# muyangyi/SimSeg

Hardware: AMD Instinct MI355X
Metric: image-text pairs/sec (train) + seg images/sec (eval), ViT-B (higher is better)
Workload: dtype fp16

## Files before the change

include/simseg_hip.h:

```cpp
#ifndef SIMSEG_HIP_H
#define SIMSEG_HIP_H
#include <stdint.h>
#ifdef __cplusplus
extern "C" {
#endif

int simseg_version(void);
int simseg_set_half_type(int t);
const char* simseg_last_error(void);

int simseg_gemm(const void* A, const void* B, void* C, int64_t M, int64_t N, int64_t K, int64_t lda, int64_t ldb,
                int64_t ldc, int in_dtype, int out_dtype, int transA, int transB, float alpha, const float* bias,
                const float* rowscale, const float* residual, int64_t ldr, int act, const void* aux, void* aux_out,
                int row_group, int res_mod, int accumulate, int splitk, uint64_t drop_seed, float drop_p, float* colsum,
                void* stream);
int simseg_gemm_aux_blocked_ok(int64_t M, int64_t N, int64_t K);

int simseg_patch_text_sim(const void* x, const void* text, float* out, int64_t M, int64_t C, int64_t K, int dtype, float eps,
                          int normalize, void* stream);

int simseg_set_gemm_variant(int v);
int simseg_gemm_last_variant(void);

int simseg_gemm_wgrad_group(const int64_t* problems, int n, int64_t rows, int slices, void* stream);
int simseg_wgrad_group_last(void);

int simseg_layernorm_fwd(const float* x, const float* gamma, const float* beta, void* y, int out_dtype, void* y_bf16,
                         float* mean, float* rstd, int64_t rows, int64_t D, float eps, void* stream);
int simseg_layernorm_bwd(const void* dy_bf16, const float* dy_f32, const float* dres, const void* dres_bf16, const float* x,
                         const void* y_bf16, const float* beta, const float* mean,
                         const float* rstd, const float* gamma, float* dx_f32, void* dx_bf16, float* dgamma,
                         float* dbeta, float* dxsum, float* partials, int64_t rows, int64_t D, uint64_t drop_seed, float drop_p,
                         void* stream);
int64_t simseg_layernorm_bwd_workspace_bytes(int64_t rows, int64_t D);

int simseg_colsum_accum(const void* in, int in_dtype, float* out, int64_t rows, int64_t N, int64_t ld, void* stream);

int simseg_vit_im2col(const float* image, void* cols, int out_dtype, int64_t B, int64_t H, int64_t W, void* stream);
int simseg_vit_cls_rows(const float* cls, const float* pos, float* x, int64_t B, int64_t T, int64_t D, void* stream);
int simseg_vit_cls_grad(const float* dx, float* dcls, int64_t B, int64_t T, int64_t D, void* stream);

int simseg_bert_embed_fwd(const int64_t* ids, const float* word, const float* pos, const float* type0, float* out,
                          int64_t B, int64_t L, int64_t D, int64_t vocab, void* stream);
int simseg_bert_embed_bwd(const int64_t* ids, const int64_t* mask, const float* dsum, float* dword, int64_t B, int64_t L,
                          int64_t D, int64_t vocab, void* stream);

int simseg_topk_pool_l2norm_fwd(const void* tok, int dtype, const int64_t* mask, float* emb, int32_t* idx, float* norm,
                                float* scratch, int64_t B, int64_t N, int64_t P, int k, float eps, int normalize, void* stream);
int64_t simseg_topk_pool_workspace_bytes(int64_t B, int64_t P, int k);
int simseg_topk_pool_l2norm_bwd(const float* demb, const float* emb, const float* norm, const int32_t* idx, void* dtok,
                                int dtype, int64_t B, int64_t N, int64_t P, int k, float eps, int normalize, void* stream);

int simseg_set_attention_variant(int v);
int simseg_debug_attn_trace(void* buf);
int simseg_debug_gemm_trace(void* buf);

// ... 153 lines not shown
```

simseg_amd/csrc/half_names.h:

```cpp
#pragma once
#ifdef SS_HALF
#define simseg_gemm_last_variant simseg_gemm_last_variant_h16
#define simseg_debug_gemm_trace simseg_debug_gemm_trace_h16
#define simseg_set_gemm_variant simseg_set_gemm_variant_h16
#define simseg_patch_text_sim simseg_patch_text_sim_h16
#define simseg_gemm_aux_blocked_ok simseg_gemm_aux_blocked_ok_h16
#define simseg_wgrad_group_last simseg_wgrad_group_last_h16
#define simseg_gemm_wgrad_group simseg_gemm_wgrad_group_h16
#define simseg_gemm simseg_gemm_h16
#define simseg_colsum_accum simseg_colsum_accum_h16
#define simseg_debug_attn_trace simseg_debug_attn_trace_h16
#define simseg_set_attention_variant simseg_set_attention_variant_h16
#define simseg_attention_fwd simseg_attention_fwd_h16
#define simseg_attention_fwd_qscaled simseg_attention_fwd_qscaled_h16
#define simseg_attention_fwd_x3 simseg_attention_fwd_x3_h16
#define simseg_debug_attention_timeline simseg_debug_attention_timeline_h16
#define simseg_attention_bwd_workspace_bytes simseg_attention_bwd_workspace_bytes_h16
#define simseg_attention_bwd simseg_attention_bwd_h16
#define simseg_attention_fwd_rows simseg_attention_fwd_rows_h16
#define simseg_attention_bwd_rows simseg_attention_bwd_rows_h16
#define simseg_attention_fwd_planes simseg_attention_fwd_planes_h16
#define simseg_attention_bwd_planes simseg_attention_bwd_planes_h16
#define simseg_layernorm_fwd simseg_layernorm_fwd_h16
#define simseg_layernorm_bwd simseg_layernorm_bwd_h16
#define simseg_layernorm_bwd_workspace_bytes simseg_layernorm_bwd_workspace_bytes_h16
#define simseg_vit_im2col simseg_vit_im2col_h16
#define simseg_topk_pool_workspace_bytes simseg_topk_pool_workspace_bytes_h16
#define simseg_topk_pool_l2norm_fwd simseg_topk_pool_l2norm_fwd_h16
#define simseg_topk_pool_l2norm_bwd simseg_topk_pool_l2norm_bwd_h16
#define simseg_row_rnorm simseg_row_rnorm_h16
#define simseg_cast simseg_cast_h16
#define simseg_dropout_apply simseg_dropout_apply_h16
#else
extern "C" {
int simseg_gemm_last_variant_h16(void);
int simseg_debug_gemm_trace_h16(void* buf);
int simseg_set_gemm_variant_h16(int v);
int simseg_patch_text_sim_h16(const void* x, const void* text, float* out, int64_t M, int64_t C, int64_t K, int dtype, float eps, int normalize, void* stream);
int simseg_gemm_aux_blocked_ok_h16(int64_t M, int64_t N, int64_t K);
int simseg_wgrad_group_last_h16(void);
int simseg_gemm_wgrad_group_h16(const int64_t* problems, int n, int64_t rows, int slices, void* stream);
int simseg_gemm_h16(const void* A, const void* B, void* C, int64_t M, int64_t N, int64_t K, int64_t lda, int64_t ldb, int64_t ldc, int in_dtype, int out_dtype, int transA, int transB, float alpha, const float* bias, const float* rowscale, const float* residual, int64_t ldr, int act, const void* aux, void* aux_out, int row_group, int res_mod, int accumulate, int splitk, uint64_t drop_seed, float drop_p, float* colsum, void* stream);
int simseg_colsum_accum_h16(const void* in, int in_dtype, float* out, int64_t rows, int64_t N, int64_t ld, void* stream);
int simseg_debug_attn_trace_h16(void* buf);
int simseg_set_attention_variant_h16(int v);
int simseg_attention_fwd_h16(const void* qkv, const int64_t* key_mask, void* out, float* lse, int dtype, int64_t B, int64_t T, int64_t H, float scale, uint64_t drop_seed, float drop_p, int skip_padded_rows, void* stream);
int simseg_attention_fwd_qscaled_h16(const void* qkv, void* out, float* lse, int64_t B, int64_t T, int64_t H, void* stream);
int simseg_attention_fwd_x3_h16(const void* qkv3, int64_t plane_elems, float* out, int64_t B, int64_t T, int64_t H, float scale, void* stream);
int simseg_debug_attention_timeline_h16(const void* qkv, void* out, float* lse, void* dbg, int64_t B, int64_t T, int64_t H, void* stream);
int64_t simseg_attention_bwd_workspace_bytes_h16(int64_t B, int64_t T, int64_t H);
int simseg_attention_bwd_h16(const void* qkv, const int64_t* key_mask, const void* out, const void* dout, const float* lse, float* workspace, void* dqkv, float* dqkv_colsum, int dtype, int64_t B, int64_t T, int64_t H, float scale, uint64_t drop_seed, float drop_p, int skip_padded_rows, void* stream);
int simseg_attention_fwd_rows_h16(const void* qkv, const int32_t* row_start, void* out, float* lse, int64_t B, int64_t T, int64_t H, float scale, uint64_t drop_seed, float drop_p, void* stream);
int simseg_attention_bwd_rows_h16(const void* qkv, const int32_t* row_start, const void* out, const void* dout, const float* lse, float* workspace, void* dqkv, float* dqkv_colsum, int64_t B, int64_t T, int64_t H, float scale, uint64_t drop_seed, float drop_p, void* stream);
int simseg_attention_fwd_planes_h16(const void* qkv, int64_t plane_rows, const int32_t* row_start, void* out, float* lse, int64_t B, int64_t T, int64_t H, float scale, uint64_t drop_seed, float drop_p, void* stream);
int simseg_attention_bwd_planes_h16(const void* qkv, int64_t plane_rows, const int32_t* row_start, const void* out, const void* dout, const float* lse, float* workspace, void* dqkv, float* dqkv_colsum, int64_t B, int64_t T, int64_t H, float scale, uint64_t drop_seed, float drop_p, void* stream);
int simseg_layernorm_fwd_h16(const float* x, const float* gamma, const float* beta, void* y, int out_dtype, void* y_bf16, float* mean, float* rstd, int64_t rows, int64_t D, float eps, void* stream);
int simseg_layernorm_bwd_h16(const void* dy_bf16, const float* dy_f32, const float* dres, const void* dres_bf16, const float* x, const void* y_bf16, const float* beta, const float* mean, const float* rstd, const float* gamma, float* dx_f32, void* dx_bf16, float* dgamma, float* dbeta, float* dxsum, float* partials, int64_t rows, int64_t D, uint64_t drop_seed, float drop_p, void* stream);
int64_t simseg_layernorm_bwd_workspace_bytes_h16(int64_t rows, int64_t D);
int simseg_vit_im2col_h16(const float* image, void* cols, int out_dtype, int64_t B, int64_t H, int64_t W, void* stream);
int64_t simseg_topk_pool_workspace_bytes_h16(int64_t B, int64_t P, int k);
int simseg_topk_pool_l2norm_fwd_h16(const void* tok, int dtype, const int64_t* mask, float* emb, int32_t* idx, float* norm, float* scratch, int64_t B, int64_t N, int64_t P, int k, float eps, int normalize, void* stream);
int simseg_topk_pool_l2norm_bwd_h16(const float* demb, const float* emb, const float* norm, const int32_t* idx, void* dtok, int dtype, int64_t B, int64_t N, int64_t P, int k, float eps, int normalize, void* stream);
int simseg_row_rnorm_h16(const void* x, int dtype, float* rnorm, int64_t rows, int64_t D, float eps, void* stream);
int simseg_cast_h16(const void* in, void* out, int64_t n, int to_bf16, void* stream);
int simseg_dropout_apply_h16(void* g, int dtype, int64_t n, uint64_t seed, float p, void* stream);
}
#endif
```

simseg_amd/csrc/rowops.hip:

```cpp
#include "common.h"
#include <atomic>
#include <stdlib.h>

namespace {

constexpr int LN_MAXC = 8;

typedef float f32x4_nt __attribute__((ext_vector_type(4)));
__device__ __forceinline__ void load4_nt(const float* p, float (&v)[4]) {
    const f32x4_nt t = __builtin_nontemporal_load(reinterpret_cast<const f32x4_nt*>(p));
    v[0] = t[0]; v[1] = t[1]; v[2] = t[2]; v[3] = t[3];
}
__device__ __forceinline__ void store4_nt(float* p, const float (&v)[4]) {
    const f32x4_nt t = {v[0], v[1], v[2], v[3]};
    __builtin_nontemporal_store(t, reinterpret_cast<f32x4_nt*>(p));
}

template <typename TO>
__global__ __launch_bounds__(256) void ln_fwd_kernel(const float* __restrict__ x, const float* __restrict__ gamma,
                                                     const float* __restrict__ beta, TO* __restrict__ y,
                                                     bf16_t* __restrict__ y2, float* __restrict__ mean_out,
                                                     float* __restrict__ rstd_out, int rows, int D, float eps) {
    const int lane = threadIdx.x & 63;
    const int row = __builtin_amdgcn_readfirstlane(blockIdx.x * 4 + (threadIdx.x >> 6));
// ... 369 lines not shown
                red[1][wave * 256 + lane * 4 + j] = ab[i][j];
                red[2][wave * 256 + lane * 4 + j] = as[i][j];
            }
        }
        __syncthreads();
        if (wave == 0 && (FULL || c < nch)) {
#pragma unroll
            for (int j = 0; j < 4; ++j) {
                float sg = 0.f, sb = 0.f, ss = 0.f;
                for (int w = 0; w < 4; ++w) { sg += red[0][w * 256 + lane * 4 + j]; sb += red[1][w * 256 + lane * 4 + j]; ss += red[2][w * 256 + lane * 4 + j]; }
                if (partials) {
                    float* pb = partials + (long)blockIdx.x * 3 * D + c * 4 + j;
                    pb[0] = sg; pb[D] = sb; pb[2 * D] = ss;
                } else {
                    atomicAdd(dgamma + c * 4 + j, sg);
                    atomicAdd(dbeta + c * 4 + j, sb);
                    if (dxsum) atomicAdd(dxsum + c * 4 + j, ss);
                }
            }
        }
    }
}

__global__ __launch_bounds__(256) void ln_bwd_reduce_kernel(const float* __restrict__ partials, int nblocks, int D, float* __restrict__ dgamma,
                                                            float* __restrict__ dbeta, float* __restrict__ dxsum) {
    const int col = blockIdx.x * 256 + threadIdx.x;
    if (col >= 3 * D) return;
    float* dst = col < D ? dgamma + col : (col < 2 * D ? dbeta + (col - D) : (dxsum ? dxsum + (col - 2 * D) : nullptr));
    if (!dst) return;
    const int per = (nblocks + gridDim.y - 1) / gridDim.y;
    const int b0 = blockIdx.y * per, b1 = min(nblocks, b0 + per);
    float s0 = 0.f, s1 = 0.f, s2 = 0.f, s3 = 0.f;
    int b = b0;
    for (; b + 4 <= b1; b += 4) {
        s0 += partials[(long)b * 3 * D + col];
        s1 += partials[(long)(b + 1) * 3 * D + col];
        s2 += partials[(long)(b + 2) * 3 * D + col];
        s3 += partials[(long)(b + 3) * 3 * D + col];
    }
    for (; b < b1; ++b) s0 += partials[(long)b * 3 * D + col];
    if (b1 > b0) atomicAdd(dst, (s0 + s1) + (s2 + s3));
}

template <typename TI>
__global__ __launch_bounds__(256) void colsum_kernel(const TI* __restrict__ in, float* __restrict__ out, long rows, int N,
                                                     long ld, int rows_per_block) {
// ... 216 lines not shown

__global__ void cast_f32_bf16_kernel(const float* __restrict__ in, bf16_t* __restrict__ out, long n4) {
    for (long i = (long)blockIdx.x * blockDim.x + threadIdx.x; i < n4; i += (long)gridDim.x * blockDim.x) {
        float v[4];
        load4<float>(in + i * 4, v);
        store4<bf16_t>(out + i * 4, v);
    }
}
__global__ void cast_bf16_f32_kernel(const bf16_t* __restrict__ in, float* __restrict__ out, long n4) {
    for (long i = (long)blockIdx.x * blockDim.x + threadIdx.x; i < n4; i += (long)gridDim.x * blockDim.x) {
        float v[4];
        load4<bf16_t>(in + i * 4, v);
        store4<float>(out + i * 4, v);
    }
}

template <typename T>
__global__ void dropout_apply_kernel(T* __restrict__ g, long n, unsigned long long seed, unsigned int thresh, float scale) {
    for (long i = (long)blockIdx.x * blockDim.x + threadIdx.x; i < n; i += (long)gridDim.x * blockDim.x)
        g[i] = (T)(dropout_keep(seed, (unsigned long long)i, thresh) ? (float)g[i] * scale : 0.f);
}

constexpr int LN_BWD_MAX_GRID = 2048;
inline int ln_bwd_grid(const void* fn, int slot, size_t lds, long rows) {
    constexpr int MAXDEV = 16;
    static std::atomic<int> ncu[MAXDEV];
    static std::atomic<unsigned long long> cached[MAXDEV][32];
    static std::atomic<int> forced{-1};
    int dev = 0;
    if (hipGetDevice(&dev) != hipSuccess || dev < 0 || dev >= MAXDEV) dev = 0;
    int n_cu = ncu[dev].load(std::memory_order_relaxed);
    if (n_cu <= 0) {
        n_cu = 256;
        hipDeviceProp_t prop;
        if (hipGetDeviceProperties(&prop, dev) == hipSuccess && prop.multiProcessorCount > 0) n_cu = prop.multiProcessorCount;
        ncu[dev].store(n_cu, std::memory_order_relaxed);
    }
    int f = forced.load(std::memory_order_relaxed);
    if (f < 0) {
        const char* e = getenv("SIMSEG_LN_BWD_BLOCKS_PER_CU");
        const int v = e ? atoi(e) : 0;
        f = v > 0 ? v : 0;
        forced.store(f, std::memory_order_relaxed);
    }
    const bool ok = slot >= 0 && slot < 32;
    const unsigned long long ent = ok ? cached[dev][slot].load(std::memory_order_relaxed) : 0ull;
    int per_cu = (ent != 0 && (ent >> 8) == (unsigned long long)lds) ? (int)(ent & 0xff) : 0;
    if (per_cu <= 0) {
        if (hipOccupancyMaxActiveBlocksPerMultiprocessor(&per_cu, fn, 256, lds) != hipSuccess || per_cu <= 0) { (void)hipGetLastError(); per_cu = 4; }
        if (per_cu > 255) per_cu = 255;
        if (ok) cached[dev][slot].store(((unsigned long long)lds << 8) | (unsigned long long)per_cu, std::memory_order_relaxed);
    }
    if (f > 0) per_cu = f;
    const long per_dev = (long)per_cu * n_cu;
    const int want = grid_for(rows, 4, LN_BWD_MAX_GRID);
    return want < per_dev ? want : (int)per_dev;
}

}

#define STREAM ((hipStream_t)stream)

extern "C" int simseg_layernorm_fwd(const float* x, const float* gamma, const float* beta, void* y, int out_dtype,
                                    void* y_bf16, float* mean, float* rstd, int64_t rows, int64_t D, float eps, void* stream) {
    SS_HALF_FWD(simseg_layernorm_fwd, x, gamma, beta, y, out_dtype, y_bf16, mean, rstd, rows, D, eps, stream);
    SS_CHECK(x && gamma && beta && y, "layernorm_fwd: null pointer");
    SS_CHECK(D % 4 == 0 && D <= LN_MAXC * 256 && D > 0, "layernorm_fwd: D=%lld must be a multiple of 4 and <= %d", (long long)D, LN_MAXC * 256);
    if (rows <= 0) return 0;
// ... 39 lines not shown
    } while (0)
#define LN_BWD16_LAUNCH(C, F)                                                                                                         \
    do {                                                                                                                              \
        grid = ln_bwd_grid((const void*)ln_bwd16_kernel<C, F>, C * 3 + (F ? 1 : 2), lds, rows);                                       \
        hipLaunchKernelGGL((ln_bwd16_kernel<C, F>), dim3(grid), dim3(256), lds, STREAM, (const bf16_t*)dy_bf16, (const bf16_t*)dres_bf16, x, (const bf16_t*)y_bf16, beta, mean, rstd, gamma, \
                           (bf16_t*)dx_bf16, dgamma, dbeta, dxsum, partials, (int)rows, (int)D, (unsigned long long)drop_seed, thresh, scale); \
    } while (0)
#define LN_BWD_PICK(C) do { if (!fast) LN_BWD_LAUNCH(C); else if (D == (C) * 256) LN_BWD16_LAUNCH(C, true); else LN_BWD16_LAUNCH(C, false); } while (0)
    if (nc <= 1) LN_BWD_PICK(1);
    else if (nc == 2) LN_BWD_PICK(2);
    else if (nc == 3) LN_BWD_PICK(3);
    else if (nc == 4) LN_BWD_PICK(4);
    else LN_BWD_PICK(8);
#undef LN_BWD_PICK
#undef LN_BWD16_LAUNCH
#undef LN_BWD_LAUNCH
    if (partials)
        hipLaunchKernelGGL(ln_bwd_reduce_kernel, dim3((unsigned)((3 * D + 255) / 256), 32), dim3(256), 0, STREAM, partials, grid, (int)D,
                           dgamma, dbeta, dxsum);
    SS_LAUNCH_CHECK("layernorm_bwd");
    return 0;
}

extern "C" int64_t simseg_layernorm_bwd_workspace_bytes(int64_t rows, int64_t D) { return (int64_t)grid_for(rows, 4, LN_BWD_MAX_GRID) * 3 * D * (int64_t)sizeof(float); }

extern "C" int simseg_colsum_accum(const void* in, int in_dtype, float* out, int64_t rows, int64_t N, int64_t ld, void* stream) {
    SS_HALF_FWD(simseg_colsum_accum, in, in_dtype, out, rows, N, ld, stream);
    SS_CHECK(in && out, "colsum: null pointer");
    SS_CHECK(N % 8 == 0 && ld % 8 == 0, "colsum: N and ld must be multiples of 8");
    if (rows <= 0) return 0;
    int chunks = (int)((rows + 255) / 256);
    if (chunks > 512) chunks = 512;
    const int nbx = (int)((N + 255) / 256);
    if ((long)chunks * nbx < 512) {
        const long by_rows = (rows + 7) / 8, by_grid = (512 + nbx - 1) / nbx;
        chunks = (int)(by_rows < by_grid ? by_rows : by_grid);
    }
    const int rpb = (int)((rows + chunks - 1) / chunks);
    dim3 grid((unsigned)nbx, (unsigned)((rows + rpb - 1) / rpb));
    if (in_dtype == 0)
        hipLaunchKernelGGL(colsum_kernel<float>, grid, dim3(256), 0, STREAM, (const float*)in, out, (long)rows, (int)N, (long)ld, rpb);
    else
        hipLaunchKernelGGL(colsum_kernel<bf16_t>, grid, dim3(256), 0, STREAM, (const bf16_t*)in, out, (long)rows, (int)N, (long)ld, rpb);
    SS_LAUNCH_CHECK("colsum");
    return 0;
}
// ... 109 lines not shown
```

simseg_amd/ops.py:

```python
import ctypes
import os
import threading

import torch

from .lib import call, ptr, require_gpu, stream, raw

F32, BF16 = 0, 1
_DT = {torch.float32: F32, torch.bfloat16: BF16, torch.float16: BF16}
HALF_TYPES = (torch.bfloat16, torch.float16)


def dt(t):
    try:
        return _DT[t.dtype]
    except KeyError:
        raise TypeError(f"simseg_amd supports fp32, bf16 and fp16 tensors, got {t.dtype}")


def _c(t):
    if t is not None and not t.is_contiguous():
        raise ValueError("simseg_amd ops need contiguous tensors")
    return t

# ... 155 lines not shown
    y16 = torch.empty(x.shape, device=x.device, dtype=want_bf16_copy if isinstance(want_bf16_copy, torch.dtype) else torch.bfloat16) if want_bf16_copy else None
    mean = torch.empty(rows, device=x.device, dtype=torch.float32) if save_stats else None
    rstd = torch.empty(rows, device=x.device, dtype=torch.float32) if save_stats else None
    call("simseg_layernorm_fwd", ptr(_c(x)), ptr(gamma), ptr(beta), ptr(y), dt(y), ptr(y16), ptr(mean), ptr(rstd), rows, D,
         float(eps), stream())
    return y, y16, mean, rstd


def layernorm_bwd(x, mean, rstd, gamma, dgamma, dbeta, dy16=None, dy32=None, dres=None, want_f32=True, want_bf16=True,
                  dxsum=None, drop_seed=0, drop_p=0.0, dres16=None, y16=None, beta=None):
    require_gpu(x)
    D = x.shape[-1]
    rows = x.numel() // D
    dx32 = torch.empty(x.shape, device=x.device, dtype=torch.float32) if want_f32 else None
    h16 = dy16.dtype if dy16 is not None else (want_bf16 if isinstance(want_bf16, torch.dtype) else torch.bfloat16)
    dx16 = torch.empty(x.shape, device=x.device, dtype=h16) if want_bf16 else None
    partials = torch.empty(raw("simseg_layernorm_bwd_workspace_bytes", rows, D) // 4, device=x.device, dtype=torch.float32)
    call("simseg_layernorm_bwd", ptr(_c(dy16)), ptr(_c(dy32)), ptr(_c(dres)), ptr(_c(dres16)), ptr(_c(x)), ptr(_c(y16)), ptr(_c(beta)) if y16 is not None else None,
         ptr(mean), ptr(rstd), ptr(gamma),
         ptr(dx32), ptr(dx16), ptr(dgamma), ptr(dbeta), ptr(dxsum), ptr(partials), rows, D, int(drop_seed), float(drop_p), stream())
    return dx32, dx16


def colsum_accum(x2d, out):
    require_gpu(x2d)
    call("simseg_colsum_accum", ptr(_c(x2d)), dt(x2d), ptr(out), x2d.shape[0], x2d.shape[1], x2d.shape[1], stream())
    return out


def vit_im2col(image, out_dtype):
    require_gpu(image)
    B, C, H, W = image.shape
    if C != 3 or image.dtype != torch.float32:
        raise ValueError("vit_im2col expects fp32 [B,3,H,W]")
    cols = torch.empty(B * (H // 16) * (W // 16), 768, device=image.device, dtype=out_dtype)
    call("simseg_vit_im2col", ptr(_c(image)), ptr(cols), dt(cols), B, H, W, stream())
    return cols


def vit_cls_rows(cls, pos, x):
    B, T, D = x.shape
    call("simseg_vit_cls_rows", ptr(cls), ptr(pos), ptr(x), B, T, D, stream())


def vit_cls_grad(dx, dcls):
    B, T, D = dx.shape
# ... 755 lines not shown
```

simseg_amd/towers.py:

```python
import contextlib
import os
import weakref

import torch
from torch.autograd import Function

from . import ops

BF16, F32 = torch.bfloat16, torch.float32


_W16 = {}


def weights_rewritten(param, w16):
    _W16[id(param)] = (weakref.ref(param), param._version, param.data_ptr(), w16)
    _W3.pop(id(param), None)
    for key in _WQS_OF.pop(id(param), ()):
        _WQS.pop(key, None)


def invalidate_weight_cache():
    _W16.clear()
    _CAT.clear()
# ... 127 lines not shown
        return cat
    return torch.cat(parts)


def _splitk(m, n, k_rows):
    tiles = ((m + 127) // 128) * ((n + 127) // 128)
    nk = (k_rows + 63) // 64
    return max(1, min(nk, (1024 + tiles - 1) // tiles, 64))


def _zeros(device, *shapes):
    sizes = [int(torch.Size(sh).numel()) if not isinstance(sh, int) else sh for sh in shapes]
    offs, o = [], 0
    for n in sizes:
        offs.append(o)
        o += (n + 63) // 64 * 64
    buf = torch.zeros(o, device=device, dtype=F32)
    return [buf[a:a + n].view(sh) for a, n, sh in zip(offs, sizes, shapes)]


_GELU8 = os.environ.get("SIMSEG_AMD_GELU_GRAD_BITS", "8") != "16"
_RES16 = os.environ.get("SIMSEG_AMD_RESGRAD_BITS", "16") != "32"
_XHAT_Y = os.environ.get("SIMSEG_AMD_LN_BWD_FROM_OUTPUT", "1") != "0"


def _lazy32(shape, device, dx16, dsum):
    dx = torch.empty(shape, device=device, dtype=F32)
    dx._simseg_lazy32 = True
    _put_shadow(dx, dx16.view(shape), dsum)
    return dx


def _need_shadow(t32, sh):
    if sh is None and getattr(t32, "_simseg_lazy32", False):
        raise RuntimeError("a residual-stream gradient that exists only as its 16-bit shadow (SIMSEG_AMD_RESGRAD_BITS=16) reached a consumer without a "
                           "valid shadow - was it modified in place, or consumed twice?  Set SIMSEG_AMD_RESGRAD_BITS=32")


def _grad_target(p):
    f = getattr(p, "_simseg_grad_target", None)
    return f() if f is not None else None


def _zeros_or(device, targets, *shapes):
    use = [t is not None and tuple(t.shape) == tuple(torch.Size(sh if not isinstance(sh, int) else (sh,))) for t, sh in zip(targets, shapes)]
    rest = iter(_zeros(device, *[sh for sh, u in zip(shapes, use) if not u]))
# ... 464 lines not shown
    try:
        mask._simseg_ragged = (mask._version, multiple, plan)
    except Exception:
        pass
    return plan


def ragged_maps(mask, multiple=256):
    p = ragged_plan(mask, multiple)
    return p.idx, p.inv, p.nv


def ragged_rows(mask):
    return ragged_plan(mask).cu


_PACKED_ATTN = os.environ.get("SIMSEG_AMD_PACKED_ATTN", "1") != "0"


class BertLayerFn(_GradAwareFn):

    @staticmethod
    def forward(ctx, x, mask, heads, adt, drop_p, seed, qw, qb, kw, kb, vw, vb, ow, ob, law, lab, iw, ib, o2w, o2b, low, lob, idx=None, inv=None,
                cu=None, nv=0):
        packed = idx is not None
        B, L = mask.shape
        D = x.shape[-1]
        x = x.contiguous()
        save = _saving(ctx)
        sh16 = getattr(x, "_simseg_fwd16", None) if adt != F32 else None
        if sh16 is not None and sh16[1] == x._version and sh16[0].numel() == x.numel():
            xa = sh16[0].view(-1, D)
        else:
            xa = x.view(-1, D) if adt == F32 else ops.cast(x.view(-1, D), adt)
        wqkv = _wt_stacked((qw, kw, vw), adt)
        bqkv = _as_one(qb.detach(), kb.detach(), vb.detach())
        if bqkv is None:
            bqkv = torch.cat([qb.detach(), kb.detach(), vb.detach()])
        ow_, iw_, o2w_ = _wt(ow, adt), _wt(iw, adt), _wt(o2w, adt)
        qkv = ops.gemm(xa, wqkv, bias=bqkv)
        rows = packed and cu is not None and adt != F32
        if rows:
            att, lse = ops.attention_fwd_rows(qkv, heads, cu, L, scale=64 ** -0.5, save_lse=save, drop_seed=seed, drop_p=drop_p, n_real=nv)
            attd = None
        else:
            if packed:
                qkv = ops.gather_rows(qkv, inv)
            att, lse = ops.attention_fwd(qkv.view(B, L, 3 * D), heads, mask, scale=64 ** -0.5, save_lse=save, drop_seed=seed, drop_p=drop_p,
                                          skip_padded_rows=packed and _SKIP_PAD, zero_skipped=False)
            attd = att
            if packed:
                att = ops.gather_rows(att.view(-1, D), idx)
        s1 = _fwd_gemm(att.view(-1, D), ow, adt, save, bias=ob.detach(), residual=x.view(-1, D), out_dtype=F32, drop_seed=seed + 1, drop_p=drop_p)
        a32, a16, mean_a, rstd_a = ops.layernorm_fwd(s1, law.detach(), lab.detach(), 1e-12, want_bf16_copy=(adt if adt != F32 else False), save_stats=save)
        aa = a32 if adt == F32 else a16
        blk = save and adt != F32 and ops.gemm_aux_blocked_ok(aa.shape[0], iw.shape[0], D)
        g8 = blk and _GELU8
        pre = torch.empty(x.shape[0] if packed else B * L, iw.shape[0], device=x.device, dtype=torch.uint8 if g8 else adt) if save else None
        act = _fwd_gemm(aa, iw, adt, save, bias=ib.detach(), act=((7 if g8 else 5) if blk else 3) if save else 1, aux_out=pre)
        s2 = _fwd_gemm(act, o2w, adt, save, bias=o2b.detach(), residual=a32, out_dtype=F32, drop_seed=seed + 2, drop_p=drop_p)
        y, y16, mean_o, rstd_o = ops.layernorm_fwd(s2, low.detach(), lob.detach(), 1e-12, want_bf16_copy=(adt if (adt != F32 and packed) else False), save_stats=save)
        if y16 is not None:
            y._simseg_fwd16 = (y16, y._version)
        ctx.adt, ctx.heads, ctx.dims, ctx.drop, ctx.packed, ctx.rows, ctx.nv, ctx.blk = adt, heads, (B, L, D), (drop_p, seed), packed, rows, nv, (2 if g8 else 1) if blk else 0
        ctx.wparams = (o2w, iw, ow)
        if save:
            ctx.save_for_backward(xa, mask, qkv, att, lse, s1, mean_a, rstd_a, aa, pre, act, s2, mean_o, rstd_o, wqkv, ow_, iw_, o2w_,
                                  law.detach(), low.detach(), attd if (packed and not rows) else None, idx, inv, cu if rows else None)
        return y if packed else y.view(B, L, D)

    @staticmethod
    @_joins_wgrad
    def backward(ctx, dy):
        (xa, mask, qkv, att, lse, s1, mean_a, rstd_a, aa, pre, act, s2, mean_o, rstd_o, wqkv, ow_, iw_, o2w_, law, low, attd, idx, inv, cu) = ctx.saved_tensors
        B, L, D = ctx.dims
        packed = ctx.packed
        adt = ctx.adt
        p, seed = ctx.drop
        need = ctx.needs_input_grad
        dy = dy.contiguous().view(-1, D)
        I = pre.shape[1]
        tg = [_grad_target(w) if nd else None for w, nd in zip(ctx.wparams, (need[18], need[16], need[12]))]
        (dlow, dlob, do2b, dib, do2w_z, diw_z, dlaw, dlab, dob, dow_z, dwqkv_z, dbqkv_z) = _zeros_or(
            dy.device, (None, None, None, None, tg[0], tg[1], None, None, None, tg[2], None, None),
            (D,), (D,), (D,), (I,), (D, I), (I, D), (D,), (D,), (D,), (D, D), (3 * D, D), (3 * D,))
        ds2_32, d2 = _ln_bwd(adt, s2, mean_o, rstd_o, low, dlow, dlob, None if adt != F32 else dy, dy32=dy if adt != F32 else None,
                             dxsum=do2b, drop=(p, seed + 2))
        group = [] if _wgrad_grouped(adt, (need[18], need[16], need[12], need[6] or need[8] or need[10])) else None
        wg = _wgrad if group is None else (lambda d, x_, z: group.append((d, x_, z)) or z)
        dpre = _dgrad(d2, o2w_, act=(4, 6, 8)[ctx.blk], aux=pre, colsum=dib)
        do2w = wg(d2, act, do2w_z) if need[18] else None
        da = _dgrad(dpre, iw_) if adt != F32 else _dgrad(dpre, iw_, residual=ds2_32)
        diw = wg(dpre, aa, diw_z) if need[16] else None
        ds1_32, d1 = _ln_bwd(adt, s1, mean_a, rstd_a, law, dlaw, dlab, da, dy32=ds2_32 if adt != F32 else None, dxsum=dob,
                             drop=(p, seed + 1))
        datt = _dgrad(d1, ow_)
        dow = wg(d1, att.view(-1, D), dow_z) if need[12] else None
        dbqkv = _zeros_like_bias(dbqkv_z, 3 * D, qkv.device) if (need[7] or need[9] or need[11]) else None
        if ctx.rows:
            dqkv = ops.attention_bwd_rows(qkv, att, datt.contiguous(), lse, ctx.heads, cu, L, scale=64 ** -0.5, drop_seed=seed, drop_p=p,
                                          colsum=dbqkv if _FUSED_QKV_BIAS else None, n_real=ctx.nv)
        else:
            if packed:
                datt = ops.gather_rows(datt, inv)
            dqkv = ops.attention_bwd(qkv.view(B, L, 3 * D), (attd if packed else att).view(B, L, D), datt.view(B, L, D), lse, ctx.heads, mask,
                                     scale=64 ** -0.5, drop_seed=seed, drop_p=p, skip_padded_rows=packed and _SKIP_PAD,
                                     colsum=dbqkv if _FUSED_QKV_BIAS else None, zero_skipped=False).view(-1, 3 * D)
            if packed:
                dqkv = ops.gather_rows(dqkv, idx)
        if dbqkv is not None and not _FUSED_QKV_BIAS:
            ops.colsum_accum(dqkv, dbqkv)
        dx = _dgrad(dqkv, wqkv, residual=ds1_32, out_dtype=F32)
        dwqkv = wg(dqkv, xa, dwqkv_z) if (need[6] or need[8] or need[10]) else None
        if group:
            _wgrad_flush(group)
        dws = [dwqkv[i * D:(i + 1) * D] if dwqkv is not None else None for i in range(3)]
        dbs = [dbqkv[i * D:(i + 1) * D] if dbqkv is not None else None for i in range(3)]
        return (dx if packed else dx.view(B, L, D), None, None, None, None, None, dws[0], dbs[0], dws[1], dbs[1], dws[2], dbs[2], dow, dob,
                dlaw, dlab, diw, dib, do2w, do2b, dlow, dlob, None, None, None, None)


_PACK_TEXT = [False, None]
_SKIP_PAD = os.environ.get("SIMSEG_AMD_SKIP_PAD_ROWS", "1") != "0"


@contextlib.contextmanager
def packed_text(lengths=None):
    prev = list(_PACK_TEXT)
    _PACK_TEXT[0] = os.environ.get("SIMSEG_AMD_PACKED_TEXT", "1") != "0"
    _PACK_TEXT[1] = lengths
    try:
        yield
    finally:
        _PACK_TEXT[:] = prev


def bert_forward(m, input_ids, attention_mask, adt, training=False, seed=0):
    p_h = m.hidden_dropout_prob if training else 0.0
    p_a = m.attention_probs_dropout_prob if training else 0.0
    if p_h != p_a:
        raise NotImplementedError("hidden and attention dropout probabilities are expected to be equal (HF default 0.1)")
    e = m.embeddings
    mask = attention_mask.contiguous().long()
    x = BertEmbedFn.apply(input_ids, mask, e.word_embeddings.weight, e.position_embeddings.weight, e.token_type_embeddings.weight,
                          e.LayerNorm.weight, e.LayerNorm.bias, p_h, seed)
    B, L, D = x.shape
    idx = inv = cu = None
    nv = 0
    if _PACK_TEXT[0] and x.is_cuda:
        lengths = _PACK_TEXT[1]
        plan = ragged_plan(mask, lengths=lengths if (lengths is not None and len(lengths) == B) else None)
        idx, inv, nv = plan.idx, plan.inv, plan.nv
        if nv == 0 or idx.numel() >= B * L:
            idx = inv = None
        else:
            x = RowMapFn.apply(x.view(-1, D), idx, inv)
            if _PACKED_ATTN and adt != F32 and L <= 256:
                cu = plan.cu
    for i, lyr in enumerate(m.encoder.layer):
        a, s = lyr.attention, lyr.attention.self
        x = BertLayerFn.apply(x, mask, m.num_heads, adt, p_h, seed + 16 * (i + 1),
                              s.query.weight, s.query.bias, s.key.weight, s.key.bias, s.value.weight, s.value.bias,
                              a.output.dense.weight, a.output.dense.bias, a.output.LayerNorm.weight, a.output.LayerNorm.bias,
                              lyr.intermediate.dense.weight, lyr.intermediate.dense.bias,
                              lyr.output.dense.weight, lyr.output.dense.bias, lyr.output.LayerNorm.weight, lyr.output.LayerNorm.bias,
                              idx, inv, cu, nv)
    if idx is not None:
        x = RowMapFn.apply(x, inv, idx).view(B, L, D)
    return x


_SKIP_MASKS = {}


def _skip_mask(B, N, skip, device):
    key = (B, N, skip, str(device))
    m = _SKIP_MASKS.get(key)
    if m is None:
        if len(_SKIP_MASKS) > 16:
            _SKIP_MASKS.clear()
        m = torch.ones(B, N, device=device, dtype=torch.int64)
        m[:, :skip] = 0
        _SKIP_MASKS[key] = m
    return m


class ProjectPoolFn(_GradAwareFn):

    @staticmethod
# ... 32 lines not shown
```

Before: 6150.

## Carry BERT residual gradients in 16-bit through a fused post-LN backward kernel

Adds a LayerNorm-backward kernel that takes one or two 16-bit gradient addends (or one fp32 addend), rebuilds xhat from the saved 16-bit LN output, and writes 16-bit dx plus an optional dropout-masked copy. The packed BERT text tower uses it so residual gradients stay in 16-bit between the two LayerNorms and across layers, and the fp32 dx of layers after the first is materialized lazily. The goal is less fp32 memory traffic in text-tower backward. The cost is lower precision in residual-gradient accumulation and more code paths, including shadow-gradient plumbing between layers.

```diff
diff --git a/include/simseg_hip.h b/include/simseg_hip.h
--- a/include/simseg_hip.h
+++ b/include/simseg_hip.h
@@ -32,6 +32,10 @@
                          const float* rstd, const float* gamma, float* dx_f32, void* dx_bf16, float* dgamma,
                          float* dbeta, float* dxsum, float* partials, int64_t rows, int64_t D, uint64_t drop_seed, float drop_p,
                          void* stream);
+int simseg_layernorm_bwd_post16(const void* dy_a, const void* dy_b, const float* dy_a_f32, const float* x, const void* y_bf16, const float* beta,
+                                const float* mean, const float* rstd, const float* gamma, void* dx_bf16, void* dxm_bf16,
+                                float* dx_f32, float* dgamma, float* dbeta, float* dxsum, float* partials, int64_t rows, int64_t D,
+                                uint64_t drop_seed, float drop_p, void* stream);
 int64_t simseg_layernorm_bwd_workspace_bytes(int64_t rows, int64_t D);
 
 int simseg_colsum_accum(const void* in, int in_dtype, float* out, int64_t rows, int64_t N, int64_t ld, void* stream);
diff --git a/simseg_amd/csrc/half_names.h b/simseg_amd/csrc/half_names.h
--- a/simseg_amd/csrc/half_names.h
+++ b/simseg_amd/csrc/half_names.h
@@ -23,6 +23,7 @@
 #define simseg_attention_bwd_planes simseg_attention_bwd_planes_h16
 #define simseg_layernorm_fwd simseg_layernorm_fwd_h16
 #define simseg_layernorm_bwd simseg_layernorm_bwd_h16
+#define simseg_layernorm_bwd_post16 simseg_layernorm_bwd_post16_h16
 #define simseg_layernorm_bwd_workspace_bytes simseg_layernorm_bwd_workspace_bytes_h16
 #define simseg_vit_im2col simseg_vit_im2col_h16
 #define simseg_topk_pool_workspace_bytes simseg_topk_pool_workspace_bytes_h16
@@ -56,6 +57,7 @@
 int simseg_attention_bwd_planes_h16(const void* qkv, int64_t plane_rows, const int32_t* row_start, const void* out, const void* dout, const float* lse, float* workspace, void* dqkv, float* dqkv_colsum, int64_t B, int64_t T, int64_t H, float scale, uint64_t drop_seed, float drop_p, void* stream);
 int simseg_layernorm_fwd_h16(const float* x, const float* gamma, const float* beta, void* y, int out_dtype, void* y_bf16, float* mean, float* rstd, int64_t rows, int64_t D, float eps, void* stream);
 int simseg_layernorm_bwd_h16(const void* dy_bf16, const float* dy_f32, const float* dres, const void* dres_bf16, const float* x, const void* y_bf16, const float* beta, const float* mean, const float* rstd, const float* gamma, float* dx_f32, void* dx_bf16, float* dgamma, float* dbeta, float* dxsum, float* partials, int64_t rows, int64_t D, uint64_t drop_seed, float drop_p, void* stream);
+int simseg_layernorm_bwd_post16_h16(const void* dy_a, const void* dy_b, const float* dy_a_f32, const float* x, const void* y_bf16, const float* beta, const float* mean, const float* rstd, const float* gamma, void* dx_bf16, void* dxm_bf16, float* dx_f32, float* dgamma, float* dbeta, float* dxsum, float* partials, int64_t rows, int64_t D, uint64_t drop_seed, float drop_p, void* stream);
 int64_t simseg_layernorm_bwd_workspace_bytes_h16(int64_t rows, int64_t D);
 int simseg_vit_im2col_h16(const float* image, void* cols, int out_dtype, int64_t B, int64_t H, int64_t W, void* stream);
 int64_t simseg_topk_pool_workspace_bytes_h16(int64_t B, int64_t P, int k);
diff --git a/simseg_amd/csrc/rowops.hip b/simseg_amd/csrc/rowops.hip
--- a/simseg_amd/csrc/rowops.hip
+++ b/simseg_amd/csrc/rowops.hip
@@ -415,6 +415,158 @@
     }
 }
 
+template <int MAXC, bool FULL, int ADD>
+__global__ __launch_bounds__(256) void ln_post16_kernel(const bf16_t* __restrict__ dya, const bf16_t* __restrict__ dyb, const float* __restrict__ dya32,
+                                                        const float* __restrict__ x, const bf16_t* __restrict__ y16, const float* __restrict__ beta,
+                                                        const float* __restrict__ mean, const float* __restrict__ rstd,
+                                                        const float* __restrict__ gamma, bf16_t* __restrict__ dx16, bf16_t* __restrict__ dxm16,
+                                                        float* __restrict__ dx32, float* __restrict__ dgamma,
+                                                        float* __restrict__ dbeta, float* __restrict__ dxsum, float* __restrict__ partials,
+                                                        int rows, int D,
+                                                        unsigned long long drop_seed, unsigned int drop_thresh, float drop_scale) {
+    constexpr bool TWO = ADD == 1, A32 = ADD == 2;
+    __shared__ float red[3][1024];
+    extern __shared__ float par[];
+    const int lane = threadIdx.x & 63, wave = threadIdx.x >> 6;
+    const int nch = D >> 2;
+    float ag[MAXC][4], ab[MAXC][4], as[MAXC][4];
+    unsigned okmask = 0;
+    int off[MAXC];
+#pragma unroll
+    for (int i = 0; i < MAXC; ++i) {
+#pragma unroll
+        for (int j = 0; j < 4; ++j) { ag[i][j] = 0.f; ab[i][j] = 0.f; as[i][j] = 0.f; }
+        const int c = lane + 64 * i;
+        off[i] = (FULL || c < nch) ? c * 4 : 0;
+        if (FULL || c < nch) {
+            float gm[4], bt[4], ig[4];
+            load4<float>(gamma + c * 4, gm);
+            load4<float>(beta + c * 4, bt);
+            bool ok = true;
+#pragma unroll
+            for (int j = 0; j < 4; ++j) { ok = ok && fabsf(gm[j]) >= 0.05f && fabsf(bt[j]) <= 4.f * fabsf(gm[j]); ig[j] = 1.0f / gm[j]; }
+            if (ok) okmask |= 1u << i;
+            if (wave == 0) { store4<float>(par + c * 4, gm); store4<float>(par + D + c * 4, ig); store4<float>(par + 2 * D + c * 4, bt); }
+        } else {
+            okmask |= 1u << i;
+        }
+    }
+    const bool needx = !__all(okmask == (1u << MAXC) - 1u);
+    __syncthreads();
+    const int stride = gridDim.x * 4;
+    int row = __builtin_amdgcn_readfirstlane(blockIdx.x * 4 + wave);
+    bf16x4 rda[A32 ? 1 : MAXC], rdb[TWO ? MAXC : 1], ry[MAXC];
+    f32x4_nt rdf[A32 ? MAXC : 1];
+#define LNP16_ISSUE(R)                                                                                            \
+    do {                                                                                                          \
+        const long ro_ = (long)(R) * D;                                                                           \
+        _Pragma("unroll") for (int i = 0; i < MAXC; ++i) {                                                        \
+            if (A32) rdf[A32 ? i : 0] = __builtin_nontemporal_load(reinterpret_cast<const f32x4_nt*>(dya32 + ro_ + off[i])); \
+            else rda[A32 ? 0 : i] = __builtin_nontemporal_load(reinterpret_cast<const bf16x4*>(dya + ro_ + off[i])); \
+            if (TWO) rdb[TWO ? i : 0] = __builtin_nontemporal_load(reinterpret_cast<const bf16x4*>(dyb + ro_ + off[i])); \
+            ry[i] = __builtin_nontemporal_load(reinterpret_cast<const bf16x4*>(y16 + ro_ + off[i]));              \
+        }                                                                                                         \
+    } while (0)
+    if (row < rows) LNP16_ISSUE(row);
+    for (; row < rows; row += stride) {
+        const float rs = rstd[row];
+        const long ro = (long)row * D;
+        float g[MAXC][4], xh[MAXC][4];
+        float s1 = 0.f, s2 = 0.f;
+        asm volatile("" ::: "memory");
+        if (needx) {
+            const float mu = mean[row];
+#pragma unroll
+            for (int i = 0; i < MAXC; ++i)
+                if (!((okmask >> i) & 1u)) {
+                    load4_nt(x + ro + off[i], xh[i]);
+#pragma unroll
+                    for (int j = 0; j < 4; ++j) xh[i][j] = (xh[i][j] - mu) * rs;
+                }
+        }
+        __builtin_amdgcn_sched_barrier(0);
+#pragma unroll
+        for (int i = 0; i < MAXC; ++i) {
+            const int c = lane + 64 * i;
+            const bool valid = FULL || c < nch;
+            const bool fromy = !needx || ((okmask >> i) & 1u);
+            float gm[4], ig[4], bt[4];
+            if (i) __builtin_amdgcn_sched_barrier(0);
+            load4<float>(par + off[i], gm);
+            load4<float>(par + D + off[i], ig);
+            load4<float>(par + 2 * D + off[i], bt);
+#pragma unroll
+            for (int j = 0; j < 4; ++j) {
+                const float sum = A32 ? rdf[A32 ? i : 0][j] : (TWO ? (float)rda[A32 ? 0 : i][j] + (float)rdb[TWO ? i : 0][j] : (float)rda[A32 ? 0 : i][j]);
+                const float a = valid ? sum : 0.f;
+                const float fy = ((float)ry[i][j] - bt[j]) * ig[j];
+                xh[i][j] = valid ? (fromy ? fy : xh[i][j]) : 0.f;
+                ag[i][j] += a * xh[i][j];
+                ab[i][j] += a;
+                g[i][j] = a * gm[j];
+                s1 += g[i][j];
+                s2 += g[i][j] * xh[i][j];
+            }
+        }
+        __builtin_amdgcn_sched_barrier(0);
+        { const int nr = row + stride < rows ? row + stride : row; LNP16_ISSUE(nr); }
+        __builtin_amdgcn_sched_barrier(0);
+        s1 = wave_sum_uniform(s1) / D;
+        s2 = wave_sum_uniform(s2) / D;
+#pragma unroll
+        for (int i = 0; i < MAXC; ++i) {
+            const int c = lane + 64 * i;
+            const bool valid = FULL || c < nch;
+            float out[4];
+#pragma unroll
+            for (int j = 0; j < 4; ++j) out[j] = rs * (g[i][j] - s1 - xh[i][j] * s2);
+            if (valid) {
+                store4<bf16_t>(dx16 + ro + off[i], out);
+                if (dx32) store4_nt(dx32 + ro + off[i], out);
+            }
+            if (drop_thresh) {
+#pragma unroll
+                for (int j = 0; j < 4; ++j) out[j] = dropout_keep(drop_seed, (unsigned long long)(ro + off[i]) + j, drop_thresh) ? out[j] * drop_scale : 0.f;
+                if (valid) store4<bf16_t>(dxm16 + ro + off[i], out);
+            }
+            if (valid) {
+#pragma unroll
+                for (int j = 0; j < 4; ++j) as[i][j] += out[j];
+            }
+        }
+    }
+#undef LNP16_ISSUE
+#pragma unroll
+    for (int i = 0; i < MAXC; ++i) {
+        const int c = lane + 64 * i;
+        __syncthreads();
+        if (FULL || c < nch) {
+#pragma unroll
+            for (int j = 0; j < 4; ++j) {
+                red[0][wave * 256 + lane * 4 + j] = ag[i][j];
+                red[1][wave * 256 + lane * 4 + j] = ab[i][j];
+                red[2][wave * 256 + lane * 4 + j] = as[i][j];
+            }
+        }
+        __syncthreads();
+        if (wave == 0 && (FULL || c < nch)) {
+#pragma unroll
+            for (int j = 0; j < 4; ++j) {
+                float sg = 0.f, sb = 0.f, ss = 0.f;
+                for (int w = 0; w < 4; ++w) { sg += red[0][w * 256 + lane * 4 + j]; sb += red[1][w * 256 + lane * 4 + j]; ss += red[2][w * 256 + lane * 4 + j]; }
+                if (partials) {
+                    float* pb = partials + (long)blockIdx.x * 3 * D + c * 4 + j;
+                    pb[0] = sg; pb[D] = sb; pb[2 * D] = ss;
+                } else {
+                    atomicAdd(dgamma + c * 4 + j, sg);
+                    atomicAdd(dbeta + c * 4 + j, sb);
+                    if (dxsum) atomicAdd(dxsum + c * 4 + j, ss);
+                }
+            }
+        }
+    }
+}
+
 __global__ __launch_bounds__(256) void ln_bwd_reduce_kernel(const float* __restrict__ partials, int nblocks, int D, float* __restrict__ dgamma,
                                                             float* __restrict__ dbeta, float* __restrict__ dxsum) {
     const int col = blockIdx.x * 256 + threadIdx.x;
@@ -677,10 +829,11 @@
 }
 
 constexpr int LN_BWD_MAX_GRID = 2048;
+constexpr int LN_BWD_SLOTS = 96;
 inline int ln_bwd_grid(const void* fn, int slot, size_t lds, long rows) {
     constexpr int MAXDEV = 16;
     static std::atomic<int> ncu[MAXDEV];
-    static std::atomic<unsigned long long> cached[MAXDEV][32];
+    static std::atomic<unsigned long long> cached[MAXDEV][LN_BWD_SLOTS];
     static std::atomic<int> forced{-1};
     int dev = 0;
     if (hipGetDevice(&dev) != hipSuccess || dev < 0 || dev >= MAXDEV) dev = 0;
@@ -698,7 +851,7 @@
         f = v > 0 ? v : 0;
         forced.store(f, std::memory_order_relaxed);
     }
-    const bool ok = slot >= 0 && slot < 32;
+    const bool ok = slot >= 0 && slot < LN_BWD_SLOTS;
     const unsigned long long ent = ok ? cached[dev][slot].load(std::memory_order_relaxed) : 0ull;
     int per_cu = (ent != 0 && (ent >> 8) == (unsigned long long)lds) ? (int)(ent & 0xff) : 0;
     if (per_cu <= 0) {
@@ -784,6 +937,48 @@
     return 0;
 }
 
+extern "C" int simseg_layernorm_bwd_post16(const void* dy_a, const void* dy_b, const float* dy_a_f32, const float* x, const void* y_bf16, const float* beta,
+                                           const float* mean, const float* rstd, const float* gamma, void* dx_bf16, void* dxm_bf16,
+                                           float* dx_f32, float* dgamma, float* dbeta, float* dxsum, float* partials, int64_t rows, int64_t D,
+                                           uint64_t drop_seed, float drop_p, void* stream) {
+    SS_HALF_FWD(simseg_layernorm_bwd_post16, dy_a, dy_b, dy_a_f32, x, y_bf16, beta, mean, rstd, gamma, dx_bf16, dxm_bf16, dx_f32, dgamma, dbeta, dxsum, partials, rows, D, drop_seed, drop_p, stream);
+    SS_CHECK(x && y_bf16 && beta && mean && rstd && gamma && dgamma && dbeta && dx_bf16, "layernorm_bwd_post16: null pointer");
+    SS_CHECK((dy_a != nullptr) != (dy_a_f32 != nullptr) && !(dy_a_f32 && dy_b), "layernorm_bwd_post16: one or two 16-bit addends, or one fp32 addend");
+    SS_CHECK(D % 4 == 0 && D <= LN_MAXC * 256 && D > 0, "layernorm_bwd_post16: bad D=%lld", (long long)D);
+    SS_CHECK(drop_p >= 0.f && drop_p < 1.f, "layernorm_bwd_post16: dropout p out of range");
+    SS_CHECK((drop_p > 0.f) == (dxm_bf16 != nullptr), "layernorm_bwd_post16: the masked output goes with a dropout mask (p > 0), and only with one");
+    if (rows <= 0) return 0;
+    const unsigned int thresh = drop_p > 0.f ? (unsigned int)((double)drop_p * 4294967296.0) : 0u;
+    SS_CHECK((drop_p > 0.f) == (thresh != 0u), "layernorm_bwd_post16: dropout p too small for the 32-bit threshold");
+    const float scale = drop_p > 0.f ? 1.0f / (1.0f - drop_p) : 1.0f;
+    const int nc = (int)((D + 255) / 256);
+    const size_t lds = (size_t)3 * D * sizeof(float);
+    int grid = 0;
+#define LN_POST_LAUNCH(C, F, A)                                                                                                       \
+    do {                                                                                                                              \
+        grid = ln_bwd_grid((const void*)ln_post16_kernel<C, F, A>, 32 + (C * 2 + (F ? 1 : 0)) * 3 + A, lds, rows);                    \
+        hipLaunchKernelGGL((ln_post16_kernel<C, F, A>), dim3(grid), dim3(256), lds, STREAM, (const bf16_t*)dy_a, (const bf16_t*)dy_b, dy_a_f32, x, (const bf16_t*)y_bf16, beta, mean, rstd, \
+                           gamma, (bf16_t*)dx_bf16, (bf16_t*)dxm_bf16, dx_f32, dgamma, dbeta, dxsum, partials, (int)rows, (int)D, (unsigned long long)drop_seed, thresh, scale); \
+    } while (0)
+#define LN_POST_PICK(C)                                                                                                               \
+    do {                                                                                                                              \
+        if (D == (C) * 256) { if (dy_a_f32) LN_POST_LAUNCH(C, true, 2); else if (dy_b) LN_POST_LAUNCH(C, true, 1); else LN_POST_LAUNCH(C, true, 0); } \
+        else { if (dy_a_f32) LN_POST_LAUNCH(C, false, 2); else if (dy_b) LN_POST_LAUNCH(C, false, 1); else LN_POST_LAUNCH(C, false, 0); } \
+    } while (0)
+    if (nc <= 1) LN_POST_PICK(1);
+    else if (nc == 2) LN_POST_PICK(2);
+    else if (nc == 3) LN_POST_PICK(3);
+    else if (nc == 4) LN_POST_PICK(4);
+    else LN_POST_PICK(8);
+#undef LN_POST_PICK
+#undef LN_POST_LAUNCH
+    if (partials)
+        hipLaunchKernelGGL(ln_bwd_reduce_kernel, dim3((unsigned)((3 * D + 255) / 256), 32), dim3(256), 0, STREAM, partials, grid, (int)D,
+                           dgamma, dbeta, dxsum);
+    SS_LAUNCH_CHECK("layernorm_bwd_post16");
+    return 0;
+}
+
 extern "C" int64_t simseg_layernorm_bwd_workspace_bytes(int64_t rows, int64_t D) { return (int64_t)grid_for(rows, 4, LN_BWD_MAX_GRID) * 3 * D * (int64_t)sizeof(float); }
 
 extern "C" int simseg_colsum_accum(const void* in, int in_dtype, float* out, int64_t rows, int64_t N, int64_t ld, void* stream) {
diff --git a/simseg_amd/ops.py b/simseg_amd/ops.py
--- a/simseg_amd/ops.py
+++ b/simseg_amd/ops.py
@@ -201,6 +201,25 @@
     return dx32, dx16
 
 
+def layernorm_bwd_post16(x, y16, beta, mean, rstd, gamma, dgamma, dbeta, dya, dyb=None, dxsum=None, drop_seed=0, drop_p=0.0, want_f32=False):
+    require_gpu(x)
+    D = x.shape[-1]
+    rows = x.numel() // D
+    a32 = dya.dtype == torch.float32
+    h16 = y16.dtype
+    if h16 not in HALF_TYPES or (not a32 and dya.dtype != h16) or (dyb is not None and (dyb.dtype != h16 or a32)):
+        raise TypeError("layernorm_bwd_post16: y16 and one or two 16-bit addends of its type, or one fp32 addend")
+    if dya.numel() != x.numel() or y16.numel() != x.numel() or (dyb is not None and dyb.numel() != x.numel()):
+        raise ValueError("layernorm_bwd_post16: dya, dyb and y16 must have the shape of x")
+    dx16 = torch.empty(x.shape, device=x.device, dtype=h16)
+    dxm16 = torch.empty(x.shape, device=x.device, dtype=h16) if drop_p > 0 else None
+    dx32 = torch.empty(x.shape, device=x.device, dtype=torch.float32) if want_f32 else None
+    partials = torch.empty(raw("simseg_layernorm_bwd_workspace_bytes", rows, D) // 4, device=x.device, dtype=torch.float32)
+    call("simseg_layernorm_bwd_post16", None if a32 else ptr(_c(dya)), ptr(_c(dyb)), ptr(_c(dya)) if a32 else None, ptr(_c(x)), ptr(_c(y16)), ptr(_c(beta)), ptr(mean), ptr(rstd), ptr(gamma),
+         ptr(dx16), ptr(dxm16), ptr(dx32), ptr(dgamma), ptr(dbeta), ptr(dxsum), ptr(partials), rows, D, int(drop_seed), float(drop_p), stream())
+    return dx16, (dxm16 if dxm16 is not None else dx16), dx32
+
+
 def colsum_accum(x2d, out):
     require_gpu(x2d)
     call("simseg_colsum_accum", ptr(_c(x2d)), dt(x2d), ptr(out), x2d.shape[0], x2d.shape[1], x2d.shape[1], stream())
diff --git a/simseg_amd/towers.py b/simseg_amd/towers.py
--- a/simseg_amd/towers.py
+++ b/simseg_amd/towers.py
@@ -173,6 +173,8 @@
 _GELU8 = os.environ.get("SIMSEG_AMD_GELU_GRAD_BITS", "8") != "16"
 _RES16 = os.environ.get("SIMSEG_AMD_RESGRAD_BITS", "16") != "32"
 _XHAT_Y = os.environ.get("SIMSEG_AMD_LN_BWD_FROM_OUTPUT", "1") != "0"
+_POST16 = os.environ.get("SIMSEG_AMD_TEXT_RESGRAD_BITS", "16") != "32"
+TEXT_RES16_LAYERS = [0]
 
 
 def _lazy32(shape, device, dx16, dsum):
@@ -683,7 +685,7 @@
 
     @staticmethod
     def forward(ctx, x, mask, heads, adt, drop_p, seed, qw, qb, kw, kb, vw, vb, ow, ob, law, lab, iw, ib, o2w, o2b, low, lob, idx=None, inv=None,
-                cu=None, nv=0):
+                cu=None, nv=0, lazy_ok=False):
         packed = idx is not None
         B, L = mask.shape
         D = x.shape[-1]
@@ -725,36 +727,57 @@
             y._simseg_fwd16 = (y16, y._version)
         ctx.adt, ctx.heads, ctx.dims, ctx.drop, ctx.packed, ctx.rows, ctx.nv, ctx.blk = adt, heads, (B, L, D), (drop_p, seed), packed, rows, nv, (2 if g8 else 1) if blk else 0
         ctx.wparams = (o2w, iw, ow)
+        ctx.t16 = bool(save and packed and adt != F32 and _POST16 and _XHAT_Y and y16 is not None)
+        ctx.lazy = ctx.t16 and bool(lazy_ok)
         if save:
             ctx.save_for_backward(xa, mask, qkv, att, lse, s1, mean_a, rstd_a, aa, pre, act, s2, mean_o, rstd_o, wqkv, ow_, iw_, o2w_,
-                                  law.detach(), low.detach(), attd if (packed and not rows) else None, idx, inv, cu if rows else None)
+                                  law.detach(), low.detach(), attd if (packed and not rows) else None, idx, inv, cu if rows else None,
+                                  *((y16, lab.detach(), lob.detach()) if ctx.t16 else ()))
         return y if packed else y.view(B, L, D)
 
     @staticmethod
     @_joins_wgrad
     def backward(ctx, dy):
-        (xa, mask, qkv, att, lse, s1, mean_a, rstd_a, aa, pre, act, s2, mean_o, rstd_o, wqkv, ow_, iw_, o2w_, law, low, attd, idx, inv, cu) = ctx.saved_tensors
+        (xa, mask, qkv, att, lse, s1, mean_a, rstd_a, aa, pre, act, s2, mean_o, rstd_o, wqkv, ow_, iw_, o2w_, law, low, attd, idx, inv, cu) = ctx.saved_tensors[:24]
         B, L, D = ctx.dims
         packed = ctx.packed
         adt = ctx.adt
         p, seed = ctx.drop
         need = ctx.needs_input_grad
-        dy = dy.contiguous().view(-1, D)
+        t16 = ctx.t16
+        dy = dy.contiguous()
+        if t16:
+            sh = _take_shadow(dy, adt)
+            if sh is not None and not (torch.is_tensor(sh[1]) and sh[1].dtype == adt and sh[1].numel() == dy.numel()):
+                sh = None
+            _need_shadow(dy, sh)
+            dya, dyb = (sh[0].view(-1, D), sh[1].view(-1, D)) if sh is not None else (dy.view(-1, D), None)
+        else:
+            _need_shadow(dy, None)
+        dy = dy.view(-1, D)
         I = pre.shape[1]
         tg = [_grad_target(w) if nd else None for w, nd in zip(ctx.wparams, (need[18], need[16], need[12]))]
         (dlow, dlob, do2b, dib, do2w_z, diw_z, dlaw, dlab, dob, dow_z, dwqkv_z, dbqkv_z) = _zeros_or(
             dy.device, (None, None, None, None, tg[0], tg[1], None, None, None, tg[2], None, None),
             (D,), (D,), (D,), (I,), (D, I), (I, D), (D,), (D,), (D,), (D, D), (3 * D, D), (3 * D,))
-        ds2_32, d2 = _ln_bwd(adt, s2, mean_o, rstd_o, low, dlow, dlob, None if adt != F32 else dy, dy32=dy if adt != F32 else None,
-                             dxsum=do2b, drop=(p, seed + 2))
+        if t16:
+            y16, lab, lob = ctx.saved_tensors[24:]
+            ds2_16, d2, _ = ops.layernorm_bwd_post16(s2, y16, lob, mean_o, rstd_o, low, dlow, dlob, dya, dyb, dxsum=do2b, drop_seed=seed + 2, drop_p=p)
+        else:
+            ds2_32, d2 = _ln_bwd(adt, s2, mean_o, rstd_o, low, dlow, dlob, None if adt != F32 else dy, dy32=dy if adt != F32 else None,
+                                 dxsum=do2b, drop=(p, seed + 2))
         group = [] if _wgrad_grouped(adt, (need[18], need[16], need[12], need[6] or need[8] or need[10])) else None
         wg = _wgrad if group is None else (lambda d, x_, z: group.append((d, x_, z)) or z)
         dpre = _dgrad(d2, o2w_, act=(4, 6, 8)[ctx.blk], aux=pre, colsum=dib)
         do2w = wg(d2, act, do2w_z) if need[18] else None
         da = _dgrad(dpre, iw_) if adt != F32 else _dgrad(dpre, iw_, residual=ds2_32)
         diw = wg(dpre, aa, diw_z) if need[16] else None
-        ds1_32, d1 = _ln_bwd(adt, s1, mean_a, rstd_a, law, dlaw, dlab, da, dy32=ds2_32 if adt != F32 else None, dxsum=dob,
-                             drop=(p, seed + 1))
+        if t16:
+            ds1_16, d1, ds1_32 = ops.layernorm_bwd_post16(s1, aa, lab, mean_a, rstd_a, law, dlaw, dlab, da, ds2_16, dxsum=dob, drop_seed=seed + 1,
+                                                          drop_p=p, want_f32=not ctx.lazy)
+        else:
+            ds1_32, d1 = _ln_bwd(adt, s1, mean_a, rstd_a, law, dlaw, dlab, da, dy32=ds2_32 if adt != F32 else None, dxsum=dob,
+                                 drop=(p, seed + 1))
         datt = _dgrad(d1, ow_)
         dow = wg(d1, att.view(-1, D), dow_z) if need[12] else None
         dbqkv = _zeros_like_bias(dbqkv_z, 3 * D, qkv.device) if (need[7] or need[9] or need[11]) else None
@@ -771,14 +794,19 @@
                 dqkv = ops.gather_rows(dqkv, idx)
         if dbqkv is not None and not _FUSED_QKV_BIAS:
             ops.colsum_accum(dqkv, dbqkv)
-        dx = _dgrad(dqkv, wqkv, residual=ds1_32, out_dtype=F32)
+        if ctx.lazy:
+            dx = _lazy32((dqkv.shape[0], D), dqkv.device, _dgrad(dqkv, wqkv), ds1_16)
+        else:
+            dx = _dgrad(dqkv, wqkv, residual=ds1_32, out_dtype=F32)
+        if t16:
+            TEXT_RES16_LAYERS[0] += 1
         dwqkv = wg(dqkv, xa, dwqkv_z) if (need[6] or need[8] or need[10]) else None
         if group:
             _wgrad_flush(group)
         dws = [dwqkv[i * D:(i + 1) * D] if dwqkv is not None else None for i in range(3)]
         dbs = [dbqkv[i * D:(i + 1) * D] if dbqkv is not None else None for i in range(3)]
         return (dx if packed else dx.view(B, L, D), None, None, None, None, None, dws[0], dbs[0], dws[1], dbs[1], dws[2], dbs[2], dow, dob,
-                dlaw, dlab, diw, dib, do2w, do2b, dlow, dlob, None, None, None, None)
+                dlaw, dlab, diw, dib, do2w, do2b, dlow, dlob, None, None, None, None, None)
 
 
 _PACK_TEXT = [False, None]
@@ -825,7 +853,7 @@
                               a.output.dense.weight, a.output.dense.bias, a.output.LayerNorm.weight, a.output.LayerNorm.bias,
                               lyr.intermediate.dense.weight, lyr.intermediate.dense.bias,
                               lyr.output.dense.weight, lyr.output.dense.bias, lyr.output.LayerNorm.weight, lyr.output.LayerNorm.bias,
-                              idx, inv, cu, nv)
+                              idx, inv, cu, nv, i > 0)
     if idx is not None:
         x = RowMapFn.apply(x, inv, idx).view(B, L, D)
     return x
```

Measured after the change: 6178 (median of 6 runs). About the same (+0.5%).
